# hjr37/diff-gaussian-rasterization

Hardware: AMD Instinct MI355X
Metric: Mviews/sec fwd+bwd @1080p, 500k Gaussians (higher is better)
Workload: dtype f32

## Files before the change

diff-gaussian-rasterization_amd/csrc/render_common.h:

```cpp
#pragma once
#include "dgr_common.h"
#include "kernels.h"
#include "wave_reduce.h"
#include "exact_math.h"

namespace dgr {

__device__ __forceinline__ uint4 blend_slot(const uint4* __restrict__ sched, const uint2* __restrict__ ranges,
                                            const uint32_t* __restrict__ sched_flag, int tiles, bool* overflowed = nullptr,
                                            bool* quadrant_lists = nullptr) {
    const int flag = __builtin_amdgcn_readfirstlane((int)*sched_flag);
    if (overflowed) *overflowed = (flag & 2) != 0;
    if (quadrant_lists) *quadrant_lists = (flag & 4) != 0;
    if (flag & 1) return sched[blockIdx.x];
    const int tile = xcd_contiguous((int)blockIdx.x, tiles);
    const uint2 r = ranges[tile];
    return make_uint4((uint32_t)tile, r.x, r.y, 0u);
}

__device__ __forceinline__ bool wave_any(bool p) { return __builtin_amdgcn_ballot_w64(p) != 0ull; }

namespace {

constexpr float LOG2E = 1.4426950408889634f, LN2 = 0.6931471805599453f;
constexpr float ALPHA_MIN = 15.0f / 255.0f;

enum { ALPHA_REF = 0, ALPHA_FAST = 1, ALPHA_GLIBC = 2 };
template <int AM>
struct AlphaPath {
    static constexpr bool LOG2 = (AM == ALPHA_FAST);
    static constexpr float PSCALE = LOG2 ? LOG2E : 1.0f;
    static constexpr float PUNSCALE = LOG2 ? LN2 : 1.0f;
    static constexpr bool TABLE = (AM == ALPHA_GLIBC);
};
template <int AM, bool UNTESTED_ARG = false>
__device__ __forceinline__ float alpha_raw(float o, float p2, const uint64_t* tab) {
    if (AM == ALPHA_FAST) return o * __builtin_amdgcn_exp2f(p2);
    if (AM == ALPHA_GLIBC) return o * exp_glibc<UNTESTED_ARG>(p2, tab);
    return o * exp_p32<UNTESTED_ARG>(p2);
}
template <int AM>
__device__ __forceinline__ float t_div(float T, float om, float& inv) {
    if (AM == ALPHA_FAST) { inv = __builtin_amdgcn_rcpf(om); return T * inv; }
    return div_ref(T, om, inv);
}

template <int NB, typename LIST_T = unsigned short, int NLISTS = 4, bool KEEP_ID = true>
struct StagedT {
    typedef LIST_T list_t;
    static constexpr bool HAS_ID = KEEP_ID;
    static constexpr int SLOTS = NB;
    static constexpr int SENTINEL = NB;
    static constexpr int LIST_LD = NB + 8;
    float4 rec[2 * (NB + 1)];
    float4 rgbd[NB + 1];
    uint32_t id[KEEP_ID ? NB : 1];
    LIST_T list[NLISTS][LIST_LD];
    int cnt4[4][NLISTS];
};
using Staged = StagedT<DGR_TILE_PIX>;

template <bool HALF_CODES>
__device__ __forceinline__ unsigned reach_code(const float4& q0, const float4& q1, float l2, float tile_x0, float tile_y0);

template <int AM, bool HALF_CODES = false, class S>
__device__ __forceinline__ unsigned stage_one(S& s, int slot, uint32_t gid, const float4* __restrict__ rec,
                                              float tile_x0, float tile_y0) {
    const float4 q0 = rec[DGR_REC_STRIDE * (size_t)gid + 0];
    const float4 q1 = rec[DGR_REC_STRIDE * (size_t)gid + 1];
    const float4 q2 = rec[DGR_REC_STRIDE * (size_t)gid + 2];
    const float o = q0.w;
    const float l2 = __log2f(o * (255.0f / 15.0f));
    constexpr float PSCALE = AlphaPath<AM>::PSCALE;
    float lthr = (o > 0.f) ? (-l2 * (AlphaPath<AM>::LOG2 ? 1.0f : LN2) - 1.0e-4f) : 3.0e38f;
    float zword = __int_as_float(slot);
    if (HALF_CODES) {
        lthr = fmaxf(lthr, -3.0e38f);
        lthr = __int_as_float(((__float_as_int(lthr) + 0xFF) & ~0xFF) | slot);
        zword = 0.f;
    }
    s.rec[2 * slot] = make_float4(q0.x, q0.y, -0.5f * PSCALE * q1.x, -0.5f * PSCALE * q1.z);
    s.rec[2 * slot + 1] = make_float4(-PSCALE * q1.y, o, zword, lthr);
    s.rgbd[slot] = make_float4(q2.x, q2.y, q2.z, q0.z);
    if (S::HAS_ID) s.id[slot] = gid;
    return reach_code<HALF_CODES>(q0, q1, l2, tile_x0, tile_y0);
}
template <bool HALF_CODES>
__device__ __forceinline__ unsigned reach_code(const float4& q0, const float4& q1, float l2, float tile_x0, float tile_y0) {
    const float tau = 2.0f * 0.6931471805599453f * l2;
    const float det = q1.x * q1.z - q1.y * q1.y;
    if (!(tau > 0.0f)) return 0u;
    if (!(det > 0.0f && q1.x > 0.0f && q1.z > 0.0f)) return HALF_CODES ? 0xFFu : 0xFu;
    const float k = tau * __builtin_amdgcn_rcpf(det);
    const float hx = __builtin_amdgcn_sqrtf(k * q1.z) * 1.001f + 0.05f, hy = __builtin_amdgcn_sqrtf(k * q1.x) * 1.001f + 0.05f;
    const float gx = q0.x - tile_x0, gy = q0.y - tile_y0;
    const bool xl = (gx + hx >= 0.0f) && (gx - hx <= 7.0f), xr = (gx + hx >= 8.0f) && (gx - hx <= 15.0f);
    if (HALF_CODES) {
        const float lo = gy - hy, hi = gy + hy;
        const unsigned xm = (xl ? 0x33u : 0u) | (xr ? 0xCCu : 0u);
        const unsigned ym = ((hi >= 0.0f) && (lo <= 3.0f) ? 0x05u : 0u) | ((hi >= 4.0f) && (lo <= 7.0f) ? 0x0Au : 0u) |
// ... 22 lines not shown

template <int AM, int TAGS, class S>
__device__ __forceinline__ unsigned stage_tagged(S& s, int slot, uint32_t entry, const float4* __restrict__ rec,
                                                 const uint8_t* __restrict__ tag8) {
    constexpr float PSCALE = AlphaPath<AM>::PSCALE;
    unsigned code = (unsigned)*tag8;
    if (code == 0u) return 0u;
    if (TAGS == TAGS_BYTES_QUADRANT) code = fold8(code);
    const uint32_t gid = entry & ID_MASK;
    const float4 q0 = rec[DGR_REC_STRIDE * (size_t)gid + 0];
    const float4 q1 = rec[DGR_REC_STRIDE * (size_t)gid + 1];
    const float4 q2 = rec[DGR_REC_STRIDE * (size_t)gid + 2];
    s.rec[2 * slot] = make_float4(q0.x, q0.y, -0.5f * PSCALE * q1.x, -0.5f * PSCALE * q1.z);
    s.rec[2 * slot + 1] = make_float4(-PSCALE * q1.y, q0.w, __int_as_float(slot * 4), __int_as_float(slot * 16));
    s.rgbd[slot] = make_float4(q2.x, q2.y, q2.z, q0.z);
    s.id[slot] = gid;
    return code;
}

__device__ __forceinline__ int lanes_below(unsigned long long m) {
    return (int)__builtin_amdgcn_mbcnt_hi((unsigned)(m >> 32), __builtin_amdgcn_mbcnt_lo((unsigned)m, 0u));
}

template <class S>
__device__ __forceinline__ int build_lists(S& s, unsigned code, int tid, int wave, int lane) {
    typedef typename S::list_t LT;
    unsigned long long bal[4];
#pragma unroll
    for (int w = 0; w < 4; w++) {
        bal[w] = __ballot((code >> w) & 1u);
        if (lane == 0) s.cnt4[wave][w] = __popcll(bal[w]);
    }
    __syncthreads();
#pragma unroll
    for (int w = 0; w < 4; w++) {
        if ((code >> w) & 1u) {
            int base = 0;
            for (int sw = 0; sw < wave; sw++) base += s.cnt4[sw][w];
            s.list[w][base + lanes_below(bal[w])] = (LT)(tid * 32);
        }
    }
    const int n = __builtin_amdgcn_readfirstlane(s.cnt4[0][wave] + s.cnt4[1][wave] + s.cnt4[2][wave] + s.cnt4[3][wave]);
    __syncthreads();
    if (lane < 4) s.list[wave][n + lane] = (LT)(S::SENTINEL * 32);
    return n;
}

template <class S>
__device__ __forceinline__ int build_half_lists(S& s, unsigned code, int tid, int wave, int lane) {
    typedef typename S::list_t LT;
    unsigned long long bal[8];
#pragma unroll
    for (int l = 0; l < 8; l++) {
        bal[l] = __ballot((code >> l) & 1u);
        if (lane == 0) s.cnt4[wave][l] = __popcll(bal[l]);
    }
    __syncthreads();
    int before = 0, all = 0;
    if (lane < 8) {
#pragma unroll
        for (int sw = 0; sw < 4; sw++) {
            const int c = s.cnt4[sw][lane];
            before += sw < wave ? c : 0;
            all += c;
        }
    }
#pragma unroll
    for (int l = 0; l < 8; l++) {
        const int base = __builtin_amdgcn_readlane(before, l);
        if ((code >> l) & 1u) s.list[l][base + lanes_below(bal[l])] = (LT)(tid * 32);
    }
    const int l0 = 2 * wave;
    const int n0 = __builtin_amdgcn_readlane(all, l0), n1 = __builtin_amdgcn_readlane(all, l0 + 1);
    __syncthreads();
    const int n = max(n0, n1);
    for (int i = n0 + lane; i < n + 4; i += 64) s.list[l0][i] = (LT)(S::SENTINEL * 32);
    for (int i = n1 + lane; i < n + 4; i += 64) s.list[l0 + 1][i] = (LT)(S::SENTINEL * 32);
    return n;
}

template <class S>
__device__ __forceinline__ int build_paired_lists(S& s, unsigned code8, int tid, int wave, int lane, unsigned long long (&split)[2]) {
    typedef typename S::list_t LT;
    static_assert(sizeof(LT) == 4 && S::SLOTS <= 128, "paired lists: 32-bit entries, at most two ranks per lane");
    unsigned long long bal[4];
#pragma unroll
    for (int w = 0; w < 4; w++) {
        bal[w] = __ballot(((code8 >> (2 * w)) & 3u) != 0u);
        if (lane == 0) s.cnt4[wave][w] = __popcll(bal[w]);
    }
    __syncthreads();
    int before = 0, all = 0;
    if (lane < 4) {
#pragma unroll
        for (int sw = 0; sw < 4; sw++) {
            const int c = s.cnt4[sw][lane];
            before += sw < wave ? c : 0;
            all += c;
        }
    }
#pragma unroll
    for (int w = 0; w < 4; w++) {
        const unsigned t = (code8 >> (2 * w)) & 3u;
        const int base = __builtin_amdgcn_readlane(before, w);
        if (t != 0u) s.list[2 * w][base + lanes_below(bal[w])] = (LT)(tid * 32) | t;
    }
    const int n = __builtin_amdgcn_readlane(all, wave);
    __syncthreads();
    LT* const LU = s.list[2 * wave];
    LT* const LL = s.list[2 * wave + 1];
    if (n <= 64) {
        const bool have = lane < n;
        const unsigned e0 = have ? LU[lane] : 0u;
        const int t0 = (int)(e0 & 3u);
        const int tm1 = __builtin_amdgcn_update_dpp(0, t0, 0x138, 0xf, 0xf, true);
        const int tm2 = __builtin_amdgcn_update_dpp(0, tm1, 0x138, 0xf, 0xf, true);
        const int tp1 = __builtin_amdgcn_update_dpp(0, t0, 0x130, 0xf, 0xf, true);
        const int tp2 = __builtin_amdgcn_update_dpp(0, tp1, 0x130, 0xf, 0xf, true);
        const bool odd = (lane & 1) != 0;
        const bool a_self = odd ? (tm1 * t0 == 2) : (t0 * tp1 == 2);
        const bool a_side = odd ? (tp1 * tp2 == 2) : (tm2 * tm1 == 2);
        const bool p2 = !a_self && !a_side && (odd ? (t0 * tp1 == 2) : (tm1 * t0 == 2));
        const bool first = odd ? p2 : a_self, second = odd ? a_self : p2;
        const unsigned long long keep = __ballot(have && !second);
        const int steps = __popcll(keep);
        if (have) {
            const int st = lanes_below(keep) - (second ? 1 : 0);
            const LT o = e0 & ~3u;
            if (first || second) {
                (t0 == 1 ? LU : LL)[st] = o;
            } else {
                LU[st] = o;
                LL[st] = o;
            }
        }
        if (lane < 4) {
            LU[steps + lane] = (LT)(S::SENTINEL * 32);
            LL[steps + lane] = (LT)(S::SENTINEL * 32);
        }
        split[0] = __ballot(lane < steps && LU[lane] != LL[lane]);
        split[1] = 0ull;
        return steps;
    }
    const LT ea = lane < n ? LU[lane] : 0u, eb = lane + 64 < n ? LU[lane + 64] : 0u;
    if (lane < n) { LU[lane] = ea & ~3u; LL[lane] = ea & ~3u; }
    if (lane + 64 < n) { LU[lane + 64] = eb & ~3u; LL[lane + 64] = eb & ~3u; }
    if (lane < 4) {
        LU[n + lane] = (LT)(S::SENTINEL * 32);
        LL[n + lane] = (LT)(S::SENTINEL * 32);
    }
    split[0] = split[1] = 0ull;
    return n;
}

typedef float f2 __attribute__((ext_vector_type(2)));

template <int AM>
__device__ __forceinline__ float pair_p2(const float4& q0, const float4& q1, f2 pxy, f2& dxy) {
    const f2 g = {q0.x, q0.y}, ac = {q0.z, q0.w};
    dxy = g - pxy;
    if (AM == ALPHA_FAST) {
        const f2 m = ac * dxy;
        const float t = __builtin_fmaf(q1.x, dxy.y, m.x);
        return __builtin_fmaf(dxy.x, t, m.y * dxy.y);
    } else {
#pragma clang fp contract(off)
        const f2 m = (ac * dxy) * dxy;
        const float B = (q1.x * dxy.x) * dxy.y;
        return (m.x + m.y) + B;
    }
}

template <class S>
__device__ __forceinline__ void load2(const S& s, int wave, int k, float4 (&q0)[2], float4 (&q1)[2]) {
    typedef typename S::list_t LT;
    unsigned off[2];
    if (sizeof(LT) == 4) {
        const uint2 pk = *reinterpret_cast<const uint2*>(&s.list[wave][k]);
        off[0] = pk.x;
        off[1] = pk.y;
    } else {
        const unsigned pk = *reinterpret_cast<const unsigned*>(&s.list[wave][k]);
        off[0] = pk & 0xffffu;
        off[1] = pk >> 16;
    }
    const char* base = reinterpret_cast<const char*>(s.rec);
#pragma unroll
    for (int u = 0; u < 2; u++) {
        q0[u] = *reinterpret_cast<const float4*>(base + off[u]);
        q1[u] = *reinterpret_cast<const float4*>(base + off[u] + 16);
    }
}


template <bool TAGGED = false, class S>
__device__ __forceinline__ void write_sentinel(S& s) {
    constexpr int NB = S::SLOTS;
    s.rec[2 * NB] = make_float4(0.f, 0.f, 0.f, 0.f);
    s.rec[2 * NB + 1] = make_float4(0.f, 0.f, __int_as_float(TAGGED ? NB * 4 : NB), TAGGED ? __int_as_float(NB * 16) : 3.0e38f);
    s.rgbd[NB] = make_float4(0.f, 0.f, 0.f, 0.f);
}

constexpr int NACC = DGR_ACC_STRIDE;
constexpr int ACC_LD = DGR_TILE_PIX + 1;

template <int NCOMP, int LD = ACC_LD>
__device__ __forceinline__ void flush_acc(const float* lds_acc, const uint32_t* ids, int cnt, float* global_acc, int tid) {
    const int comp = tid & 15;
    if (comp < NCOMP) {
        for (int r = tid >> 4; r < cnt; r += 16) {
            const float v = lds_acc[comp * LD + r];
            if (v != 0.f) atomicAdd(global_acc + (size_t)ids[r] * DGR_ACC_STRIDE + comp, v);
        }
    }
}

}
}
```

diff-gaussian-rasterization_amd/csrc/render_full.hip:

```cpp
#include "render_common.h"

namespace dgr {
namespace {

template <class S>
__device__ __forceinline__ void flush_tags(const S& s, const uint32_t* hit, uint8_t* tag8, uint32_t pos0, int tid, bool staged) {
    if (staged) tag8[pos0 + tid] = (uint8_t)tag_byte(hit[tid], __float_as_uint(s.rec[2 * tid + 1].z));
}

template <int AM>
__global__ void __launch_bounds__(256, 8) render_fwd_full_kernel(RenderFwdFullArgs a) {
    __shared__ StagedT<DGR_TILE_PIX, unsigned short, 8> s;
    __shared__ uint32_t hit[DGR_TILE_PIX];
    __shared__ int s_nvalid;
    __shared__ uint64_t exptab[32];
    if (a.rep.host && blockIdx.x == 0 && threadIdx.x == 0) report_status(a.rep, a.status);
    bool overflowed;
    const uint4 slot = blend_slot(a.sched, a.ranges, a.sched_flag, a.grid_x * a.grid_y, &overflowed);
    const int tile = (int)slot.x;
    const int tx = tile % a.grid_x, ty = tile / a.grid_x;
    const int tid = threadIdx.x, wave = tid >> 6, lane = tid & 63;
    const int px = tx * DGR_BLOCK_X + (wave & 1) * 8 + (lane & 7);
    const int py = ty * DGR_BLOCK_Y + (wave >> 1) * 8 + (lane >> 3);
    const bool inside = px < a.W && py < a.H;
// ... 54 lines not shown
                    if (first_contributor == 0) first_contributor = last_contributor;
                    if (T < 0.0001f) ub = -__builtin_inff();
                  }
                }
            }
            if (!wave_any(ub >= 0.f)) break;
        }
    }

    __syncthreads();
    if (have_flush) flush_tags(s, hit, tag8, range.x + last_base, tid, tid < total - last_base);
    for (int p = (have_flush ? last_base + DGR_TILE_PIX : 0) + tid; p < total; p += DGR_TILE_PIX) tag8[range.x + p] = 0;

    if (overflowed) {
        C0 = C1 = C2 = U = Dd = __builtin_nanf("");
    }
    if (inside) {
        const size_t N = (size_t)a.W * a.H;
        a.final_T[pix_id] = T;
        a.n_valid[pix_id] = nvalid;
        a.n_contrib[pix_id] = last_contributor;
        a.first_contrib[pix_id] = first_contributor;
        a.out_color[pix_id] = C0 + T * a.bg[0];
        a.out_color[N + pix_id] = C1 + T * a.bg[1];
        a.out_color[2 * N + pix_id] = C2 + T * a.bg[2];
        a.out_depth[pix_id] = Dd;
        a.out_uncertainty[pix_id] = U;
    }
    {
        int v = inside ? (int)nvalid : 0;
#pragma unroll
        for (int off = 32; off > 0; off >>= 1) v += __shfl_xor(v, off, 64);
        __syncthreads();
        if (lane == 0) atomicAdd(&s_nvalid, v);
        __syncthreads();
        if (tid == 0 && s_nvalid) atomicAdd(&a.status[3], s_nvalid);
    }
}

constexpr int NACC_FULL = 15;

template <bool DET>
struct StagedBwdFull {
    static constexpr int NB = DET ? 64 : 128;
    static constexpr int LD = NB + 1;
    static constexpr int PLANE = NACC_FULL * LD;
    typedef StagedT<NB, uint32_t, DET ? 4 : 8> staged_t;
    staged_t f;
    float acc[(DET ? 4 : 1) * PLANE];
    uint32_t inst[DET ? NB : 1];
    int max_last;
    uint64_t exptab[32];
};

template <int AM, bool DET = false, bool LEAN = false>
__global__ void __launch_bounds__(256, 6) render_bwd_full_kernel(RenderBwdFullArgs a) {
    typedef StagedBwdFull<DET> SB;
    constexpr int BWD_NB = SB::NB, BWD_LD = SB::LD;
    constexpr bool PAIRED = !DET;
    __shared__ SB sb;
    typename SB::staged_t& s = sb.f;
    const uint4 slot = blend_slot(a.sched, a.ranges, a.sched_flag, a.grid_x * a.grid_y);
    const int tile = (int)slot.x;
    const int tx = tile % a.grid_x, ty = tile / a.grid_x;
    const int tid = threadIdx.x, wave = tid >> 6, lane = tid & 63;
    const int px = tx * DGR_BLOCK_X + (wave & 1) * 8 + (lane & 7);
    const int py = ty * DGR_BLOCK_Y + (wave >> 1) * 8 + (lane >> 3);
    const bool inside = px < a.W && py < a.H;
    const size_t pix_id = (size_t)a.W * py + px;
    const size_t N = (size_t)a.W * a.H;
    const f2 pxy = {(float)px, (float)py};

    const uint2 range = make_uint2(slot.y, slot.z);
    const int last_contributor = inside ? (int)a.n_contrib[pix_id] : 0;
    const int first_contributor = inside ? (int)a.first_contrib[pix_id] : 0;

    if (tid == 0) {
        sb.max_last = 0;
        write_sentinel<true>(s);
    }
    if (AlphaPath<AM>::TABLE) exp_ref_table_fill(sb.exptab, tid);
    __syncthreads();
    {
        int v = last_contributor;
#pragma unroll
        for (int off = 32; off > 0; off >>= 1) v = max(v, __shfl_xor(v, off, 64));
        if (lane == 0) atomicMax(&sb.max_last, v);
    }
    __syncthreads();
    const int total = min((int)(range.y - range.x), sb.max_last);
    if (total <= 0) return;

    const float T_final = inside ? a.final_T[pix_id] : 0.f;
    float T = T_final;
    float dpix0 = 0.f, dpix1 = 0.f, dpix2 = 0.f, dL_depth = 0.f, dL_dunc = 0.f, gt_px = 0.f;
    if (inside) {
        dpix0 = a.dL_dpix[pix_id];
        dpix1 = a.dL_dpix[N + pix_id];
        dpix2 = a.dL_dpix[2 * N + pix_id];
        dL_depth = a.dL_depths[pix_id];
        if (!LEAN && a.dL_duncertainties) dL_dunc = a.dL_duncertainties[pix_id];
        gt_px = a.gt_depth[pix_id];
    }
    const float bg_term = -T_final * (a.bg[0] * dpix0 + a.bg[1] * dpix1 + a.bg[2] * dpix2);
    const float dunc2 = 2.f * dL_dunc;
    float Sc = 0.f, Sd = 0.f, Su = 0.f;
    const float ddelx_dx = 0.5f * a.W, ddely_dy = 0.5f * a.H;
    const int c16 = wave_reduce16d_comp(lane);
    const int my_comp = ((lane & 3) == 0 && c16 < NACC_FULL) ? c16 : -1;
    const uint8_t* const tag8 = half_tags(a.point_list, a.sched_flag);
    float* const my_acc = sb.acc + (DET ? wave * SB::PLANE : 0) + (my_comp >= 0 ? my_comp : 0) * BWD_LD;

    for (int hi = total; hi > 0; hi -= BWD_NB) {
        const int lo = max(0, hi - BWD_NB);
        const int cnt = hi - lo;
        __syncthreads();
        unsigned code = 0;
        if (tid < cnt) code = stage_tagged<AM, PAIRED ? TAGS_BYTES_HALVES : TAGS_BYTES_QUADRANT>(s, tid, a.point_list[range.x + lo + tid], a.rec, tag8 + (range.x + lo + tid));
        if (!DET) {
#pragma unroll
            for (int k = 0; k < NACC_FULL; k++)
                if (tid < BWD_NB) sb.acc[k * BWD_LD + tid] = 0.f;
        }
        unsigned long long split[2] = {0ull, 0ull};
        const int n = PAIRED ? build_paired_lists(s, code, tid, wave, lane, split) : build_lists(s, code, tid, wave, lane);
        const int rel_last4 = 4 * (last_contributor - lo);
        const int rel_first4 = 4 * (first_contributor - 1 - lo);

        constexpr int U = PAIRED ? 1 : 2;
        const int my_list = PAIRED ? 2 * wave + (lane >> 5) : wave;
        for (int k = ((n + U - 1) / U) * U - U; k >= 0; k -= U) {
            float4 q0[2], q1[2];
            if (U == 2) {
                load2(s, my_list, k, q0, q1);
            } else {
                const unsigned off = s.list[my_list][k];
                q0[0] = *reinterpret_cast<const float4*>(reinterpret_cast<const char*>(s.rec) + off);
                q1[0] = *reinterpret_cast<const float4*>(reinterpret_cast<const char*>(s.rec) + off + 16);
            }
#pragma unroll
            for (int u = U - 1; u >= 0; u--) {
                f2 dxy;
                const float p2 = pair_p2<AM>(q0[u], q1[u], pxy, dxy);
                const int j4 = __float_as_int(q1[u].z);
                const float oG = alpha_raw<AM, true>(q1[u].y, p2, sb.exptab);
                const bool valid = (j4 < rel_last4) & (p2 <= 0.0f) & !(oG < ALPHA_MIN);
                const float oGm = valid ? oG : 0.f;
                const float am = fminf(0.99f, oGm);
                const float4 cd = *reinterpret_cast<const float4*>(reinterpret_cast<const char*>(s.rgbd) + __float_as_int(q1[u].w));
                const float om = 1.f - am;
                float inv;
                T = t_div<AM>(T, om, inv);
                const float w = am * T;
                const float e = cd.w - gt_px;
                const float Xc = cd.x * dpix0 + cd.y * dpix1 + cd.z * dpix2, Xd = cd.w, Xu = e * e;
                const float dcol = Xc - Sc;
                const float ddep = Xd - Sd;
                float dL_dalpha = LEAN ? dcol + ddep * dL_depth : dcol + ddep * dL_depth + (Xu - Su) * dL_dunc;
                dL_dalpha *= T;
                dL_dalpha += bg_term * inv;
                Sc = am * Xc + om * Sc;
                Sd = am * Xd + om * Sd;
                if (!LEAN) Su = am * Xu + om * Su;
                const float qq = oGm * dL_dalpha;
                const float qc = oGm * (T * dcol);
                const bool front = valid & (j4 == rel_first4);
                const float fw = front ? dL_depth * w : 0.f;
                const float fq = front ? oG * (dL_depth * (T * ddep)) : 0.f;
                const float dx = dxy.x, dy = dxy.y;
                const float qdx = qq * dx, qdy = qq * dy;
                float g[16];
                g[0] = w * dpix0;
                g[1] = w * dpix1;
                g[2] = w * dpix2;
                g[3] = LEAN ? w * dL_depth : w * dL_depth + (dunc2 * w) * e;
                g[4] = qdx;
                g[5] = qdy;
                g[6] = qdx * dx;
                g[7] = qdx * dy;
                g[8] = qdy * dy;
                g[9] = qq;
                g[10] = qc * dx;
                g[11] = qc * dy;
                g[12] = fw;
                g[13] = fq * dx;
                g[14] = fq * dy;
                g[15] = 0.f;
                float tot;
                if (PAIRED) {
                    float u0, u1;
                    wave_reduce16d_head(g, u0, u1);
                    const int st = k + u;
                    if ((split[st >> 6] >> (st & 63)) & 1ull) {
                        const float r0 = quad_sum(u0), r1 = quad_sum(u1);
                        const int c0 = (lane & 3) == 0 ? wave_reduce16d_half_slot0(lane) : -1;
                        const int c1 = ((lane & 3) == 0 && wave_reduce16d_half_slot1(lane) < NACC_FULL) ? wave_reduce16d_half_slot1(lane) : -1;
                        char* const col = reinterpret_cast<char*>(sb.acc) + j4;
                        if (c0 >= 0) atomicAdd(reinterpret_cast<float*>(col + c0 * (BWD_LD * 4)), r0);
                        if (c1 >= 0) atomicAdd(reinterpret_cast<float*>(col + c1 * (BWD_LD * 4)), r1);
                        continue;
                    }
                    tot = wave_reduce16d_tail(u0, u1);
                } else {
                    tot = wave_reduce16d(g);
                }
                if (my_comp >= 0) {
                    float* const cell = reinterpret_cast<float*>(reinterpret_cast<char*>(my_acc) + j4);
                    if (DET) *cell = tot; else atomicAdd(cell, tot);
                }
            }
        }
        __syncthreads();
        if (DET && tid < BWD_NB) {
            uint32_t row = ~0u;
            if (code != 0u) {
#pragma unroll
                for (int k = 0; k < NACC_FULL; k++) {
                    float v = 0.f;
#pragma unroll
                    for (int w = 0; w < 4; w++)
                        if ((code >> w) & 1u) v += sb.acc[w * SB::PLANE + k * BWD_LD + tid];
                    sb.acc[k * BWD_LD + tid] = v;
                }
                const uint32_t gid = s.id[tid];
                const ushort4 rc = a.det_rect[gid];
                row = a.det_goff[gid] + (uint32_t)(ty - (int)rc.y) * (uint32_t)(rc.z - rc.x) + (uint32_t)(tx - (int)rc.x);
            }
            sb.inst[tid] = row;
        }
        if (DET) __syncthreads();
        if (code != 0u) {
            constexpr float UN = AlphaPath<AM>::PUNSCALE;
            const float4 r0 = s.rec[2 * tid], r1 = s.rec[2 * tid + 1];
            const float ca = r0.z * (-2.f * UN), cb = r1.x * (-UN), cc = r0.w * (-2.f * UN);
#pragma unroll
            for (int p = 0; p < 3; p++) {
                const int cx = (p == 0) ? 4 : (p == 1) ? 10 : 13, cy = cx + 1;
                const float Sx = sb.acc[cx * BWD_LD + tid], Sy = sb.acc[cy * BWD_LD + tid];
                sb.acc[cx * BWD_LD + tid] = -(ca * Sx + cb * Sy) * ddelx_dx;
                sb.acc[cy * BWD_LD + tid] = -(cc * Sy + cb * Sx) * ddely_dy;
            }
            sb.acc[6 * BWD_LD + tid] *= -0.5f;
            sb.acc[7 * BWD_LD + tid] *= -0.5f;
            sb.acc[8 * BWD_LD + tid] *= -0.5f;
            sb.acc[9 * BWD_LD + tid] *= __builtin_amdgcn_rcpf(r1.y);
        }
        __syncthreads();
        if (DET) {
            const int comp = tid & 15;
            for (int r = tid >> 4; r < cnt; r += 16) {
                const uint32_t row = sb.inst[r];
                if (row < a.det_R && comp < NACC_FULL) a.det_rows[(size_t)row * DGR_ACC_STRIDE + comp] = sb.acc[comp * BWD_LD + r];
            }
        } else {
            flush_acc<NACC_FULL, BWD_LD>(sb.acc, s.id, cnt, a.acc, tid);
        }
    }
}

}

hipError_t launch_render_fwd_full(const RenderFwdFullArgs& a, int alpha_mode, hipStream_t stream) {
    const int tiles = a.grid_x * a.grid_y;
    if (tiles <= 0) return hipSuccess;
    switch (alpha_mode) {
        case ALPHA_FAST: launch_blend(render_fwd_full_kernel<ALPHA_FAST>, dim3(tiles), dim3(256), stream, a); break;
        case ALPHA_GLIBC: launch_blend(render_fwd_full_kernel<ALPHA_GLIBC>, dim3(tiles), dim3(256), stream, a); break;
        default: launch_blend(render_fwd_full_kernel<ALPHA_REF>, dim3(tiles), dim3(256), stream, a);
    }
    return hipGetLastError();
}
hipError_t launch_render_bwd_full(const RenderBwdFullArgs& a, int alpha_mode, hipStream_t stream, bool deterministic) {
    const int tiles = a.grid_x * a.grid_y;
    if (tiles <= 0) return hipSuccess;
    const bool lean = a.dL_duncertainties == nullptr;
    if (deterministic) {
        if (lean) launch_blend(render_bwd_full_kernel<ALPHA_REF, true, true>, dim3(tiles), dim3(256), stream, a);
        else launch_blend(render_bwd_full_kernel<ALPHA_REF, true>, dim3(tiles), dim3(256), stream, a);
        return hipGetLastError();
    }
    switch (alpha_mode) {
        case ALPHA_FAST: launch_blend(render_bwd_full_kernel<ALPHA_FAST>, dim3(tiles), dim3(256), stream, a); break;
        case ALPHA_GLIBC: launch_blend(render_bwd_full_kernel<ALPHA_GLIBC>, dim3(tiles), dim3(256), stream, a); break;
        default:
            if (lean) launch_blend(render_bwd_full_kernel<ALPHA_REF, false, true>, dim3(tiles), dim3(256), stream, a);
            else launch_blend(render_bwd_full_kernel<ALPHA_REF>, dim3(tiles), dim3(256), stream, a);
    }
    return hipGetLastError();
}

}
```

diff-gaussian-rasterization_amd/csrc/render_light.hip:

```cpp
#include "render_common.h"

namespace dgr {
namespace {

constexpr int FWD_UNROLL = 2;

template <bool HALVES>
struct StagedFwd {
    typedef StagedT<DGR_TILE_PIX, unsigned short, HALVES ? 8 : 4, !HALVES> staged_t;
    staged_t f;
    float unc[DGR_TILE_PIX];
    uint32_t cnt[DGR_TILE_PIX];
    uint32_t hit[DGR_TILE_PIX];
    uint64_t exptab[32];
};


template <class SF>
__device__ __forceinline__ void flush_slot(const SF& sf, const RenderFwdLightArgs& a, uint8_t* tag8, uint32_t pos0, int tid, bool staged) {
    if (!staged) return;
    uint32_t t8;
    if constexpr (!SF::staged_t::HAS_ID) {
        t8 = tag_byte(sf.hit[tid], __float_as_uint(sf.f.rec[2 * tid + 1].z));
    } else {
// ... 82 lines not shown
                        }
                        T = test_T;
                        last_contributor = (uint32_t)(base + j + 1);
                    }
                  }
                }
            }
            if (!wave_any(ub >= 0.f)) break;
        }
    }
    __syncthreads();
    if (have_flush) flush_slot(sf, a, tag8, range.x + last_base, tid, tid < total - last_base);
    for (int p = (have_flush ? last_base + DGR_TILE_PIX : 0) + tid; p < total; p += DGR_TILE_PIX) tag8[range.x + p] = 0;

    if (overflowed) {
        C0 = C1 = C2 = weight = Dd = D_median = __builtin_nanf("");
    }
    if (inside) {
        const uint32_t N = (uint32_t)a.W * (uint32_t)a.H;
        a.n_contrib[pix_id] = last_contributor;
        a.out_color[pix_id] = C0 + T * a.bg[0];
        a.out_color[N + pix_id] = C1 + T * a.bg[1];
        a.out_color[2 * N + pix_id] = C2 + T * a.bg[2];
        a.out_alpha[pix_id] = weight;
        a.out_depth[pix_id] = Dd;
        a.out_median[pix_id] = D_median;
        a.out_depth_var[pix_id] = 0.0f;
    }
}

template <int AM>
__global__ void __launch_bounds__(256, 8) render_fwd_light_kernel(RenderFwdLightArgs a) {
    __shared__ union { StagedFwd<true> h; StagedFwd<false> q; } sf;
    if (a.rep.host && blockIdx.x == 0 && threadIdx.x == 0) report_status(a.rep, a.status);
    bool overflowed, quadrant_lists;
    const uint4 slot = blend_slot(a.sched, a.ranges, a.sched_flag, a.grid_x * a.grid_y, &overflowed, &quadrant_lists);
    if (quadrant_lists) render_fwd_light_body<AM, false>(a, sf.q, slot, overflowed);
    else render_fwd_light_body<AM, true>(a, sf.h, slot, overflowed);
}

constexpr int NACC_LIGHT = 14;

template <bool DET, bool HALVES = false>
struct StagedBwd {
    static constexpr int NB = DET ? 64 : 128;
    static constexpr int LD = NB + 1;
    static constexpr int PLANE = NACC_LIGHT * LD;
    typedef StagedT<NB, uint32_t, HALVES ? 8 : 4> staged_t;
    staged_t f;
    float acc[(DET ? 4 : 1) * PLANE];
    uint32_t inst[DET ? NB : 1];
    int max_last;
    uint64_t exptab[32];
};

template <int AM, bool DO_MAP, bool DO_POSE, bool DET, bool LEAN, bool HALVES>
__device__ __forceinline__ void render_bwd_light_body(const RenderBwdLightArgs& a, StagedBwd<DET, HALVES>& sb, const uint4 slot) {
    static_assert(!HALVES || !DET, "half-wave / paired lists: not with the deterministic kernel's planes (LDS)");
    constexpr bool PAIRED = HALVES && DO_MAP;
    typedef StagedBwd<DET, HALVES> SB;
    constexpr int BWD_NB = SB::NB, BWD_LD = SB::LD;
    typename SB::staged_t& s = sb.f;
    const int tile = (int)slot.x;
    const int tx = tile % a.grid_x, ty = tile / a.grid_x;
    const int tid = threadIdx.x, wave = tid >> 6, lane = tid & 63;
    const int px = tx * DGR_BLOCK_X + (wave & 1) * 8 + (lane & 7);
    const int py = ty * DGR_BLOCK_Y + (wave >> 1) * 8 + (lane >> 3);
    const bool inside = px < a.W && py < a.H;
    const uint32_t pix_id = (uint32_t)a.W * (uint32_t)py + (uint32_t)px;
    const uint32_t N = (uint32_t)a.W * (uint32_t)a.H;
    const float pxf = (float)px, pyf = (float)py;
    const f2 pxy = {pxf, pyf};

    const uint2 range = make_uint2(slot.y, slot.z);
    const int last_contributor = inside ? (int)a.n_contrib[pix_id] : 0;

    if (tid == 0) {
        sb.max_last = 0;
        write_sentinel<true>(s);
    }
    if (AlphaPath<AM>::TABLE) exp_ref_table_fill(sb.exptab, tid);
    __syncthreads();
    {
        int v = last_contributor;
#pragma unroll
        for (int off = 32; off > 0; off >>= 1) v = max(v, __shfl_xor(v, off, 64));
        if (lane == 0) atomicMax(&sb.max_last, v);
    }
    __syncthreads();
    const int total = min((int)(range.y - range.x), sb.max_last);
    if (total <= 0) return;

    const float T_final = inside ? (1.0f - a.alphas[pix_id]) : 0.f;
    float T = T_final;
    float dpix0 = 0.f, dpix1 = 0.f, dpix2 = 0.f, dpix_depth = 0.f, dpix_median = 0.f, dpix_var = 0.f, gt_px = 0.f;
    if (inside) {
        dpix0 = __builtin_nontemporal_load(a.dL_dpix + pix_id);
        dpix1 = __builtin_nontemporal_load(a.dL_dpix + N + pix_id);
        dpix2 = __builtin_nontemporal_load(a.dL_dpix + 2 * N + pix_id);
        dpix_depth = __builtin_nontemporal_load(a.dL_dpix_depth + pix_id);
        if (!LEAN) {
            if (a.dL_dpix_median) dpix_median = __builtin_nontemporal_load(a.dL_dpix_median + pix_id);
            if (a.dL_dpix_var) dpix_var = __builtin_nontemporal_load(a.dL_dpix_var + pix_id);
            gt_px = __builtin_nontemporal_load(a.gt_depth + pix_id);
        }
    }
    const float bg_term = -T_final * (a.bg[0] * dpix0 + a.bg[1] * dpix1 + a.bg[2] * dpix2);
    const float ddelx_dx = 0.5f * a.W, ddely_dy = 0.5f * a.H;
    float S = 0.f;
    float mid_thr = 0.5f;
    int my_comp;
    if (DO_MAP) {
        const int c = (lane >= 48) ? 12 : wave_reduce12d_comp(lane);
        my_comp = ((lane & 3) != 0 || c > 11) ? -1 : (c == 10 ? (DO_POSE ? 13 : 10) : c == 11 ? (DO_POSE ? 10 : -1) : c);
    } else if (HALVES) {
        const int c = half_reduce3_comp(lane);
        my_comp = c == 0 ? 4 : c == 1 ? 5 : c == 2 ? 13 : -1;
    } else {
        const int c = wave_reduce4_comp(lane);
        my_comp = ((lane & 15) == 0 && c < 3) ? (c == 0 ? 4 : c == 1 ? 5 : 13) : -1;
    }
    const int my_list = HALVES ? 2 * wave + (lane >> 5) : wave;
    const uint8_t* const tag8 = half_tags(a.point_list, a.sched_flag);

    float* const my_acc = sb.acc + (DET ? wave * SB::PLANE : 0) + (my_comp >= 0 ? my_comp : 0) * BWD_LD;

    for (int hi = total; hi > 0; hi -= BWD_NB) {
        const int lo = max(0, hi - BWD_NB);
        const int cnt = hi - lo;
        __syncthreads();
        unsigned code = 0;
        if (tid < cnt) code = stage_tagged<AM, HALVES ? TAGS_BYTES_HALVES : TAGS_BYTES_QUADRANT>(s, tid, a.point_list[range.x + lo + tid], a.rec, tag8 + (range.x + lo + tid));
        if (!DET) {
#pragma unroll
            for (int k = 0; k < NACC_LIGHT; k++)
                if (BWD_NB == DGR_TILE_PIX || tid < BWD_NB) sb.acc[k * BWD_LD + tid] = 0.f;
        }
        unsigned long long split[2] = {0ull, 0ull};
        const int n = PAIRED   ? build_paired_lists(s, code, tid, wave, lane, split)
                      : HALVES ? build_half_lists(s, code, tid, wave, lane)
                               : build_lists(s, code, tid, wave, lane);
        const int rel_last4 = 4 * (last_contributor - lo);

        constexpr int U = PAIRED ? 1 : 2;
        for (int k = ((n + U - 1) / U) * U - U; k >= 0; k -= U) {
            float4 q0[2], q1[2];
            if (U == 2) {
                load2(s, my_list, k, q0, q1);
            } else {
                const unsigned off = s.list[my_list][k];
                q0[0] = *reinterpret_cast<const float4*>(reinterpret_cast<const char*>(s.rec) + off);
                q1[0] = *reinterpret_cast<const float4*>(reinterpret_cast<const char*>(s.rec) + off + 16);
            }
#pragma unroll
            for (int u = U - 1; u >= 0; u--) {
                f2 dxy;
                const float p2 = pair_p2<AM>(q0[u], q1[u], pxy, dxy);
                const float dx = dxy.x, dy = dxy.y;
                const int j4 = __float_as_int(q1[u].z);
                const float oG = alpha_raw<AM, true>(q1[u].y, p2, sb.exptab);
                const bool valid = (j4 < rel_last4) & (p2 <= 0.0f) & !(oG < ALPHA_MIN);
                const float oGm = valid ? oG : 0.f;
                const float alpha = fminf(0.99f, oGm);
                const float4 cd = *reinterpret_cast<const float4*>(reinterpret_cast<const char*>(s.rgbd) + __float_as_int(q1[u].w));
                const float om = 1.f - alpha;
                float inv;
                T = t_div<AM>(T, om, inv);
                const float w = alpha * T;
                const float e = cd.w - gt_px;
                const float X = LEAN ? cd.x * dpix0 + cd.y * dpix1 + cd.z * dpix2 + cd.w * dpix_depth
                                     : cd.x * dpix0 + cd.y * dpix1 + cd.z * dpix2 + cd.w * dpix_depth + (e * e) * dpix_var;
                const float dL_dalpha = (X - S) * T + bg_term * inv;
                S = alpha * X + om * S;
                const float qq = oGm * dL_dalpha;
                const float qdx = qq * dx, qdy = qq * dy;
                const float wd = w * dpix_depth;
                float tot;
                if (DO_MAP) {
                    float gmed = 0.f;
                    if (!LEAN) {
                        const bool fire = valid & (T > mid_thr);
                        gmed = fire ? dpix_median : 0.f;
                        mid_thr = fire ? __builtin_inff() : mid_thr;
                    }
                    float g[12];
                    g[0] = w * dpix0;
                    g[1] = w * dpix1;
                    g[2] = w * dpix2;
                    g[3] = LEAN ? wd : wd + 2.f * ((dpix_var * w) * e);
                    g[4] = qdx;
                    g[5] = qdy;
                    g[6] = qdx * dx;
                    g[7] = qdx * dy;
                    g[8] = qdy * dy;
                    g[9] = qq;
                    g[10] = DO_POSE ? wd : gmed;
                    g[11] = DO_POSE ? gmed : 0.f;
                    if (PAIRED) {
                        float u0, u1;
                        wave_reduce12d_head(g, u0, u1);
                        const int st = k + u;
                        if ((split[st >> 6] >> (st & 63)) & 1ull) {
                            const float r0 = quad_sum(u0), r1 = quad_sum(u1);
                            auto comp_of = [](int slot) { return slot < 10 ? slot : slot == 10 ? (DO_POSE ? 13 : 10) : (DO_POSE ? 10 : -1); };
                            const int s1 = wave_reduce12d_half_slot1(lane);
                            const int c0 = (lane & 3) == 0 ? comp_of(wave_reduce12d_half_slot0(lane)) : -1;
                            const int c1 = ((lane & 3) == 0 && s1 >= 0) ? comp_of(s1) : -1;
                            char* const col = reinterpret_cast<char*>(sb.acc) + j4;
                            if (c0 >= 0) atomicAdd(reinterpret_cast<float*>(col + c0 * (BWD_LD * 4)), r0);
                            if (c1 >= 0) atomicAdd(reinterpret_cast<float*>(col + c1 * (BWD_LD * 4)), r1);
                            continue;
                        }
                        tot = wave_reduce12d_tail(u0, u1);
                    } else {
                        tot = wave_reduce12d(g);
                    }
                } else if (HALVES) {
                    tot = half_reduce3(qdx, qdy, wd);
                } else {
                    float g4[4] = {qdx, qdy, wd, 0.f};
                    tot = wave_reduce4(g4);
                }
                if (my_comp >= 0) {
                    float* const cell = reinterpret_cast<float*>(reinterpret_cast<char*>(my_acc) + j4);
                    if (DET) *cell = tot; else atomicAdd(cell, tot);
                }
            }
        }

        __syncthreads();
        if (DET && tid < BWD_NB) {
            uint32_t row = ~0u;
            if (code != 0u) {
#pragma unroll
                for (int k = 0; k < NACC_LIGHT; k++) {
                    const bool delivered = DO_MAP ? (k <= 9 || k == 10 || (DO_POSE && k == 13)) : (k == 4 || k == 5 || k == 13);
                    float v = 0.f;
                    if (delivered) {
#pragma unroll
                        for (int w = 0; w < 4; w++)
                            if ((code >> w) & 1u) v += sb.acc[w * SB::PLANE + k * BWD_LD + tid];
                    }
                    sb.acc[k * BWD_LD + tid] = v;
                }
                const uint32_t gid = s.id[tid];
                const ushort4 rc = a.det_rect[gid];
                row = a.det_goff[gid] + (uint32_t)(ty - (int)rc.y) * (uint32_t)(rc.z - rc.x) + (uint32_t)(tx - (int)rc.x);
            }
            sb.inst[tid] = row;
        }
        if (DET) __syncthreads();
        if (code != 0u) {
            constexpr float UN = AlphaPath<AM>::PUNSCALE;
            const float4 r0 = s.rec[2 * tid], r1 = s.rec[2 * tid + 1];
            const float ca = r0.z * (-2.f * UN), cb = r1.x * (-UN), cc = r0.w * (-2.f * UN);
            const float Sx = sb.acc[4 * BWD_LD + tid], Sy = sb.acc[5 * BWD_LD + tid];
            sb.acc[4 * BWD_LD + tid] = -(ca * Sx + cb * Sy) * ddelx_dx;
            sb.acc[5 * BWD_LD + tid] = -(cc * Sy + cb * Sx) * ddely_dy;
            if (DO_MAP) {
                sb.acc[6 * BWD_LD + tid] *= -0.5f;
                sb.acc[7 * BWD_LD + tid] *= -0.5f;
                sb.acc[8 * BWD_LD + tid] *= -0.5f;
                sb.acc[9 * BWD_LD + tid] *= __builtin_amdgcn_rcpf(r1.y);
            }
        }
        __syncthreads();
        if (DET) {
            const int comp = tid & 15;
            for (int r = tid >> 4; r < cnt; r += 16) {
                const uint32_t row = sb.inst[r];
                if (row < a.det_R && comp < NACC_LIGHT) a.det_rows[(size_t)row * DGR_ACC_STRIDE + comp] = sb.acc[comp * BWD_LD + r];
            }
        } else {
            flush_acc<NACC_LIGHT, BWD_LD>(sb.acc, s.id, cnt, a.acc, tid);
        }
    }
}

template <int AM, bool DO_MAP, bool DO_POSE, bool DET = false, bool LEAN = false, bool BY_FRAME = false>
__global__ void __launch_bounds__(256, 8) render_bwd_light_kernel(RenderBwdLightArgs a) {
    static_assert(!BY_FRAME || !DET, "the deterministic kernel walks quadrant lists");
    __shared__ union { StagedBwd<DET, BY_FRAME> h; StagedBwd<DET, false> q; } sb;
    bool quadrant_lists = true;
    const uint4 slot = blend_slot(a.sched, a.ranges, a.sched_flag, a.grid_x * a.grid_y, nullptr, BY_FRAME ? &quadrant_lists : nullptr);
    if (BY_FRAME && !quadrant_lists) render_bwd_light_body<AM, DO_MAP, DO_POSE, DET, LEAN, BY_FRAME>(a, sb.h, slot);
    else render_bwd_light_body<AM, DO_MAP, DO_POSE, DET, LEAN, false>(a, sb.q, slot);
}

__device__ __forceinline__ uint32_t rect_tiles(ushort4 r) { return (r.z > r.x && r.w > r.y) ? (uint32_t)(r.z - r.x) * (uint32_t)(r.w - r.y) : 0u; }
__global__ void __launch_bounds__(256) det_block_sums_kernel(int P, const ushort4* __restrict__ rect, uint32_t* __restrict__ blk) {
    __shared__ uint32_t red[4];
    const int g = blockIdx.x * 256 + threadIdx.x;
    uint32_t v = g < P ? rect_tiles(rect[g]) : 0u;
#pragma unroll
    for (int off = 32; off > 0; off >>= 1) v += __shfl_xor(v, off, 64);
    if ((threadIdx.x & 63) == 0) red[threadIdx.x >> 6] = v;
    __syncthreads();
    if (threadIdx.x == 0) blk[blockIdx.x] = red[0] + red[1] + red[2] + red[3];
}
__global__ void __launch_bounds__(256) det_offsets_kernel(int P, const ushort4* __restrict__ rect, const uint32_t* __restrict__ blk,
                                                          uint32_t* __restrict__ goff) {
    __shared__ uint32_t red[4], wsum[4];
    uint32_t before = 0;
    for (int b = threadIdx.x; b < (int)blockIdx.x; b += 256) before += blk[b];
#pragma unroll
    for (int off = 32; off > 0; off >>= 1) before += __shfl_xor(before, off, 64);
    if ((threadIdx.x & 63) == 0) red[threadIdx.x >> 6] = before;
    const int g = blockIdx.x * 256 + threadIdx.x;
    const uint32_t n = g < P ? rect_tiles(rect[g]) : 0u;
    uint32_t incl = n;
#pragma unroll
    for (int off = 1; off < 64; off <<= 1) {
        const uint32_t v = __shfl_up(incl, off, 64);
        if ((threadIdx.x & 63) >= off) incl += v;
    }
    if ((threadIdx.x & 63) == 63) wsum[threadIdx.x >> 6] = incl;
    __syncthreads();
    uint32_t base = red[0] + red[1] + red[2] + red[3];
    for (int w = 0; w < (int)(threadIdx.x >> 6); w++) base += wsum[w];
    if (g < P) goff[g] = base + incl - n;
}
__global__ void __launch_bounds__(256) det_gather_kernel(int P, const ushort4* __restrict__ rect, const uint32_t* __restrict__ goff,
                                                         const float* __restrict__ rows, uint32_t R, float* __restrict__ acc) {
    const int g = blockIdx.x * 16 + (threadIdx.x >> 4), comp = threadIdx.x & 15;
    if (g >= P) return;
    uint32_t n = rect_tiles(rect[g]);
    if (n == 0u) return;
    const uint32_t first = goff[g];
    if (first >= R || n > R - first) {
        acc[(size_t)g * DGR_ACC_STRIDE + comp] = __builtin_nanf("");
        return;
    }
    const float* r = rows + (size_t)first * DGR_ACC_STRIDE + comp;
    float v = 0.f;
    for (uint32_t i = 0; i < n; i++) v += r[(size_t)i * DGR_ACC_STRIDE];
    acc[(size_t)g * DGR_ACC_STRIDE + comp] = v;
}

__global__ void __launch_bounds__(64) wave_reduce_test_kernel(const float* in, float* out16, float* out12, float* out4,
                                                             int* comp16, int* comp12, int* comp4) {
    const int lane = threadIdx.x;
    float g16[16], g12[12], g4[4];
#pragma unroll
    for (int k = 0; k < 16; k++) g16[k] = in[k * 64 + lane];
#pragma unroll
    for (int k = 0; k < 12; k++) g12[k] = g16[k];
#pragma unroll
    for (int k = 0; k < 4; k++) g4[k] = g16[k];
    out16[lane] = wave_reduce16d(g16);
    out12[lane] = wave_reduce12d(g12);
    out4[lane] = wave_reduce4(g4);
    comp16[lane] = wave_reduce16d_comp(lane);
    comp12[lane] = wave_reduce12d_comp(lane);
    comp4[lane] = wave_reduce4_comp(lane);
}

__global__ void __launch_bounds__(64) half_reduce_test_kernel(const float* in, float* r0, float* r1, float* h3, int* slot0, int* slot1,
// ... 157 lines not shown
```

Measured before the change: 0.002489.

## Streamline backward render list building, accumulator clearing and flush in LDS

```diff
diff --git a/diff-gaussian-rasterization_amd/csrc/render_common.h b/diff-gaussian-rasterization_amd/csrc/render_common.h
--- a/diff-gaussian-rasterization_amd/csrc/render_common.h
+++ b/diff-gaussian-rasterization_amd/csrc/render_common.h
@@ -16,6 +16,15 @@
     const int tile = xcd_contiguous((int)blockIdx.x, tiles);
     const uint2 r = ranges[tile];
     return make_uint4((uint32_t)tile, r.x, r.y, 0u);
+}
+
+__device__ __forceinline__ int wave_max_int(int v) {
+    v = max(v, __builtin_amdgcn_update_dpp(0, v, 0xB1, 0xf, 0xf, false));
+    v = max(v, __builtin_amdgcn_update_dpp(0, v, 0x4E, 0xf, 0xf, false));
+    v = max(v, __builtin_amdgcn_update_dpp(0, v, 0x141, 0xf, 0xf, false));
+    v = max(v, __builtin_amdgcn_update_dpp(0, v, 0x140, 0xf, 0xf, false));
+    return max(max(__builtin_amdgcn_readlane(v, 0), __builtin_amdgcn_readlane(v, 16)),
+               max(__builtin_amdgcn_readlane(v, 32), __builtin_amdgcn_readlane(v, 48)));
 }
 
 __device__ __forceinline__ bool wave_any(bool p) { return __builtin_amdgcn_ballot_w64(p) != 0ull; }
@@ -204,28 +213,34 @@
 template <class S>
 __device__ __forceinline__ int build_paired_lists(S& s, unsigned code8, int tid, int wave, int lane, unsigned long long (&split)[2]) {
     typedef typename S::list_t LT;
-    static_assert(sizeof(LT) == 4 && S::SLOTS <= 128, "paired lists: 32-bit entries, at most two ranks per lane");
+    static_assert(sizeof(LT) == 4 && S::SLOTS <= 128 && S::SLOTS % 64 == 0, "paired lists: 32-bit entries, at most two ranks per lane");
+    constexpr int SW = S::SLOTS / 64;
+    const bool stager = __builtin_amdgcn_readfirstlane(wave) < SW;
     unsigned long long bal[4];
-#pragma unroll
-    for (int w = 0; w < 4; w++) {
-        bal[w] = __ballot(((code8 >> (2 * w)) & 3u) != 0u);
-        if (lane == 0) s.cnt4[wave][w] = __popcll(bal[w]);
+    if (stager) {
+#pragma unroll
+        for (int w = 0; w < 4; w++) {
+            bal[w] = __ballot(((code8 >> (2 * w)) & 3u) != 0u);
+            if (lane == 0) s.cnt4[wave][w] = __popcll(bal[w]);
+        }
     }
     __syncthreads();
     int before = 0, all = 0;
     if (lane < 4) {
 #pragma unroll
-        for (int sw = 0; sw < 4; sw++) {
+        for (int sw = 0; sw < SW; sw++) {
             const int c = s.cnt4[sw][lane];
             before += sw < wave ? c : 0;
             all += c;
         }
     }
-#pragma unroll
-    for (int w = 0; w < 4; w++) {
-        const unsigned t = (code8 >> (2 * w)) & 3u;
-        const int base = __builtin_amdgcn_readlane(before, w);
-        if (t != 0u) s.list[2 * w][base + lanes_below(bal[w])] = (LT)(tid * 32) | t;
+    if (stager) {
+#pragma unroll
+        for (int w = 0; w < 4; w++) {
+            const unsigned base = (unsigned)__builtin_amdgcn_readlane(before, w);
+            const unsigned pos = __builtin_amdgcn_mbcnt_hi((unsigned)(bal[w] >> 32), __builtin_amdgcn_mbcnt_lo((unsigned)bal[w], base));
+            if (__builtin_amdgcn_inverse_ballot_w64(bal[w])) s.list[2 * w][pos] = (LT)(tid * 32) | ((code8 >> (2 * w)) & 3u);
+        }
     }
     const int n = __builtin_amdgcn_readlane(all, wave);
     __syncthreads();
@@ -234,27 +249,23 @@
     if (n <= 64) {
         const bool have = lane < n;
         const unsigned e0 = have ? LU[lane] : 0u;
-        const int t0 = (int)(e0 & 3u);
-        const int tm1 = __builtin_amdgcn_update_dpp(0, t0, 0x138, 0xf, 0xf, true);
-        const int tm2 = __builtin_amdgcn_update_dpp(0, tm1, 0x138, 0xf, 0xf, true);
-        const int tp1 = __builtin_amdgcn_update_dpp(0, t0, 0x130, 0xf, 0xf, true);
-        const int tp2 = __builtin_amdgcn_update_dpp(0, tp1, 0x130, 0xf, 0xf, true);
-        const bool odd = (lane & 1) != 0;
-        const bool a_self = odd ? (tm1 * t0 == 2) : (t0 * tp1 == 2);
-        const bool a_side = odd ? (tp1 * tp2 == 2) : (tm2 * tm1 == 2);
-        const bool p2 = !a_self && !a_side && (odd ? (t0 * tp1 == 2) : (tm1 * t0 == 2));
-        const bool first = odd ? p2 : a_self, second = odd ? a_self : p2;
-        const unsigned long long keep = __ballot(have && !second);
+        const unsigned t0 = e0 & 3u;
+        const unsigned long long up = __ballot(t0 == 1u), low = __ballot(t0 == 2u);
+        const unsigned long long pair = (up & (low >> 1)) | (low & (up >> 1));
+        constexpr unsigned long long EVEN = 0x5555555555555555ull;
+        const unsigned long long first0 = pair & EVEN;
+        const unsigned long long first = first0 | (pair & ~EVEN & ~(first0 << 1) & ~(first0 >> 1));
+        const unsigned long long second = first << 1;
+        const unsigned long long keep = (n == 64 ? ~0ull : (1ull << n) - 1ull) & ~second;
         const int steps = __popcll(keep);
-        if (have) {
-            const int st = lanes_below(keep) - (second ? 1 : 0);
-            const LT o = e0 & ~3u;
-            if (first || second) {
-                (t0 == 1 ? LU : LL)[st] = o;
-            } else {
-                LU[st] = o;
-                LL[st] = o;
-            }
+        const unsigned long long k1 = keep >> 1;
+        const int st = (int)__builtin_amdgcn_mbcnt_hi((unsigned)(k1 >> 32), __builtin_amdgcn_mbcnt_lo((unsigned)k1, (unsigned)(keep & 1ull) - 1u));
+        const LT o = e0 & ~3u;
+        if (__builtin_amdgcn_inverse_ballot_w64(first | second)) {
+            LU[st + (t0 == 2u ? S::LIST_LD : 0)] = o;
+        } else if (__builtin_amdgcn_inverse_ballot_w64(keep)) {
+            LU[st] = o;
+            LL[st] = o;
         }
         if (lane < 4) {
             LU[steps + lane] = (LT)(S::SENTINEL * 32);
@@ -326,16 +337,30 @@
 constexpr int NACC = DGR_ACC_STRIDE;
 constexpr int ACC_LD = DGR_TILE_PIX + 1;
 
-template <int NCOMP, int LD = ACC_LD>
-__device__ __forceinline__ void flush_acc(const float* lds_acc, const uint32_t* ids, int cnt, float* global_acc, int tid) {
+template <int NCOMP, int LD>
+__device__ __forceinline__ void clear_acc(float* lds_acc, int tid) {
+    constexpr int N = NCOMP * LD, N4 = N / 4;
+#pragma unroll
+    for (int i = 0; i < N4; i += 256)
+        if (i + 256 <= N4 || i + tid < N4) reinterpret_cast<float4*>(lds_acc)[i + tid] = make_float4(0.f, 0.f, 0.f, 0.f);
+    if (tid < N % 4) lds_acc[4 * N4 + tid] = 0.f;
+}
+template <int NCOMP, int NB, int LD>
+__device__ __forceinline__ void flush_acc(float* lds_acc, const uint32_t* ids, float* global_acc, int tid) {
+    static_assert(NB % 16 == 0 && DGR_ACC_STRIDE == 16, "flush: 16 lanes per 64-byte accumulator row");
     const int comp = tid & 15;
     if (comp < NCOMP) {
-        for (int r = tid >> 4; r < cnt; r += 16) {
-            const float v = lds_acc[comp * LD + r];
-            if (v != 0.f) atomicAdd(global_acc + (size_t)ids[r] * DGR_ACC_STRIDE + comp, v);
-        }
-    }
-}
-
-}
-}
+        float* const cell = lds_acc + comp * LD + (tid >> 4);
+        const uint32_t* const id = ids + (tid >> 4);
+        char* const row0 = reinterpret_cast<char*>(global_acc + comp);
+#pragma unroll
+        for (int i = 0; i < NB / 16; i++) {
+            const float v = cell[16 * i];
+            cell[16 * i] = 0.f;
+            if (v != 0.f) atomicAdd(reinterpret_cast<float*>(row0 + (size_t)id[16 * i] * 64u), v);
+        }
+    }
+}
+
+}
+}
diff --git a/diff-gaussian-rasterization_amd/csrc/render_full.hip b/diff-gaussian-rasterization_amd/csrc/render_full.hip
--- a/diff-gaussian-rasterization_amd/csrc/render_full.hip
+++ b/diff-gaussian-rasterization_amd/csrc/render_full.hip
@@ -160,14 +160,14 @@
     if (AlphaPath<AM>::TABLE) exp_ref_table_fill(sb.exptab, tid);
     __syncthreads();
     {
-        int v = last_contributor;
-#pragma unroll
-        for (int off = 32; off > 0; off >>= 1) v = max(v, __shfl_xor(v, off, 64));
+        const int v = wave_max_int(last_contributor);
         if (lane == 0) atomicMax(&sb.max_last, v);
     }
     __syncthreads();
     const int total = min((int)(range.y - range.x), sb.max_last);
     if (total <= 0) return;
+    static_assert(offsetof(SB, acc) % 16 == 0, "clear_acc: 16-byte stores");
+    if (!DET) clear_acc<NACC_FULL, BWD_LD>(sb.acc, tid);
 
     const float T_final = inside ? a.final_T[pix_id] : 0.f;
     float T = T_final;
@@ -195,11 +195,6 @@
         __syncthreads();
         unsigned code = 0;
         if (tid < cnt) code = stage_tagged<AM, PAIRED ? TAGS_BYTES_HALVES : TAGS_BYTES_QUADRANT>(s, tid, a.point_list[range.x + lo + tid], a.rec, tag8 + (range.x + lo + tid));
-        if (!DET) {
-#pragma unroll
-            for (int k = 0; k < NACC_FULL; k++)
-                if (tid < BWD_NB) sb.acc[k * BWD_LD + tid] = 0.f;
-        }
         unsigned long long split[2] = {0ull, 0ull};
         const int n = PAIRED ? build_paired_lists(s, code, tid, wave, lane, split) : build_lists(s, code, tid, wave, lane);
         const int rel_last4 = 4 * (last_contributor - lo);
@@ -331,7 +326,7 @@
                 if (row < a.det_R && comp < NACC_FULL) a.det_rows[(size_t)row * DGR_ACC_STRIDE + comp] = sb.acc[comp * BWD_LD + r];
             }
         } else {
-            flush_acc<NACC_FULL, BWD_LD>(sb.acc, s.id, cnt, a.acc, tid);
+            flush_acc<NACC_FULL, BWD_NB, BWD_LD>(sb.acc, s.id, a.acc, tid);
         }
     }
 }
diff --git a/diff-gaussian-rasterization_amd/csrc/render_light.hip b/diff-gaussian-rasterization_amd/csrc/render_light.hip
--- a/diff-gaussian-rasterization_amd/csrc/render_light.hip
+++ b/diff-gaussian-rasterization_amd/csrc/render_light.hip
@@ -188,14 +188,14 @@
     if (AlphaPath<AM>::TABLE) exp_ref_table_fill(sb.exptab, tid);
     __syncthreads();
     {
-        int v = last_contributor;
-#pragma unroll
-        for (int off = 32; off > 0; off >>= 1) v = max(v, __shfl_xor(v, off, 64));
+        const int v = wave_max_int(last_contributor);
         if (lane == 0) atomicMax(&sb.max_last, v);
     }
     __syncthreads();
     const int total = min((int)(range.y - range.x), sb.max_last);
     if (total <= 0) return;
+    static_assert(offsetof(SB, acc) % 16 == 0, "clear_acc: 16-byte stores");
+    if (!DET) clear_acc<NACC_LIGHT, BWD_LD>(sb.acc, tid);
 
     const float T_final = inside ? (1.0f - a.alphas[pix_id]) : 0.f;
     float T = T_final;
@@ -237,11 +237,6 @@
         __syncthreads();
         unsigned code = 0;
         if (tid < cnt) code = stage_tagged<AM, HALVES ? TAGS_BYTES_HALVES : TAGS_BYTES_QUADRANT>(s, tid, a.point_list[range.x + lo + tid], a.rec, tag8 + (range.x + lo + tid));
-        if (!DET) {
-#pragma unroll
-            for (int k = 0; k < NACC_LIGHT; k++)
-                if (BWD_NB == DGR_TILE_PIX || tid < BWD_NB) sb.acc[k * BWD_LD + tid] = 0.f;
-        }
         unsigned long long split[2] = {0ull, 0ull};
         const int n = PAIRED   ? build_paired_lists(s, code, tid, wave, lane, split)
                       : HALVES ? build_half_lists(s, code, tid, wave, lane)
@@ -315,9 +310,11 @@
                             char* const col = reinterpret_cast<char*>(sb.acc) + j4;
                             if (c0 >= 0) atomicAdd(reinterpret_cast<float*>(col + c0 * (BWD_LD * 4)), r0);
                             if (c1 >= 0) atomicAdd(reinterpret_cast<float*>(col + c1 * (BWD_LD * 4)), r1);
-                            continue;
+                        } else {
+                            tot = wave_reduce12d_tail(u0, u1);
+                            if (my_comp >= 0) atomicAdd(reinterpret_cast<float*>(reinterpret_cast<char*>(my_acc) + j4), tot);
                         }
-                        tot = wave_reduce12d_tail(u0, u1);
+                        continue;
                     } else {
                         tot = wave_reduce12d(g);
                     }
@@ -378,7 +375,7 @@
                 if (row < a.det_R && comp < NACC_LIGHT) a.det_rows[(size_t)row * DGR_ACC_STRIDE + comp] = sb.acc[comp * BWD_LD + r];
             }
         } else {
-            flush_acc<NACC_LIGHT, BWD_LD>(sb.acc, s.id, cnt, a.acc, tid);
+            flush_acc<NACC_LIGHT, BWD_NB, BWD_LD>(sb.acc, s.id, a.acc, tid);
         }
     }
 }
```

After: 0.002532 (median of 6 runs). +1.7%, better.
